# nikkolasg/playsnark

Hardware: AMD Instinct MI355X
Metric: G1 scalar-muls/s (Pippenger MSM, 2^20 pts per GPU) (higher is better)
Workload: dtype i32x14 (381-bit Fp, 28-bit unsaturated limbs, Montgomery); 1 GPU; BLS12-381 G1 MSM, 2^20 points per GPU, uniform 255-bit scalars; points_per_gpu=1048576, window_bits=20, windows=13, window_table=True, window_table_bytes=1744830464, slice=32, in_flight=4

## Files before the change

### playsnark_amd/csrc/capi.hip

```cpp
#include "../../include/playsnark_hip.h"

#include <hip/hip_runtime.h>

#include <algorithm>
#include <atomic>
#include <chrono>
#include <condition_variable>
#include <functional>
#include <mutex>
#include <cstdio>
#include <cstring>
#include <future>
#include <string>
#include <thread>
#include <vector>

#include "msm.hpp"
#include "point_pass_predict.hpp"
#include "msm_batch.hpp"
#include "msm_batch_plan.hpp"
#include "msm_batch_multi_plan.hpp"
#include "quotient.hpp"
#include "lagrange.hpp"
#include "ec_spmv.hpp"
// ... 12 lines not shown
}
#define HIP_TRY(expr)                                                                            \
    do {                                                                                         \
        hipError_t _e = (expr);                                                                  \
        if (_e != hipSuccess)                                                                    \
            return fail(PS_ERR_HIP, std::string(#expr) + ": " + hipGetErrorString(_e));          \
    } while (0)

#include "scope.hpp"

extern "C" const char* ps_last_error(void) { return g_last_error.c_str(); }
#define PS_STR_(x) #x
#define PS_STR(x) PS_STR_(x)
extern "C" const char* ps_version(void) { return "playsnark_hip 0.4 (gfx950), ABI " PS_STR(PS_ABI_VERSION); }
extern "C" int ps_abi_version(void) { return PS_ABI_VERSION; }
extern "C" int ps_device_count(void) {
    int n = 0;
    if (hipGetDeviceCount(&n) != hipSuccess) return 0;
    return n;
}

struct DevBuf {
    void* p = nullptr;
    size_t cap = 0;
    DevBuf() = default;
    DevBuf(const DevBuf&) = delete;
    DevBuf& operator=(const DevBuf&) = delete;
    ~DevBuf() { release(); }
    int ensure(size_t bytes) {
        if (bytes <= cap) return PS_OK;
        release();
        size_t want = bytes + bytes / 8 + 256;
        hipError_t e = hipMalloc(&p, want);
        if (e != hipSuccess) return fail(PS_ERR_HIP, std::string("hipMalloc workspace: ") + hipGetErrorString(e));
        cap = want;
        return PS_OK;
    }
    void release() {
        if (p) (void)hipFree(p);
        p = nullptr;
        cap = 0;
    }
};

constexpr size_t PS_PINNED_SLOT = 64 * sizeof(Xyzz<Fp2>) + 16;

struct MsmWorkspace {
    int device = 0;
    hipStream_t stream = nullptr;
    hipStream_t tail = nullptr;
    hipEvent_t ev_acc_local = nullptr, ev_tail_done = nullptr, ev_sort_local = nullptr;
    bool tail_used = false;
    DevBuf counts, offs, bsum, keys, ranks, vals, sorted, buckets, parts, segs, wins, heavy, hparts, coarse;
    DevBuf perm, border;
    DevBuf mb_fold, mb_out;
    void* h_pinned = nullptr;
    size_t h_pinned_cap = 0;
    hipEvent_t ev[PS_MSM_STAGES + 1] = {};
    bool ev_valid = false;
    ~MsmWorkspace() { destroy(); }
    bool created() const { return stream != nullptr; }
    int create(int dev) {
        const int rc = [&]() -> int {
            device = dev;
            HIP_TRY(hipSetDevice(device));
            HIP_TRY(hipStreamCreateWithFlags(&stream, hipStreamNonBlocking));
            int least = 0, greatest = 0;
            HIP_TRY(hipDeviceGetStreamPriorityRange(&least, &greatest));
            HIP_TRY(hipStreamCreateWithPriority(&tail, hipStreamNonBlocking, greatest));
            HIP_TRY(hipEventCreateWithFlags(&ev_acc_local, hipEventDisableTiming));
            HIP_TRY(hipEventCreateWithFlags(&ev_tail_done, hipEventDisableTiming));
            HIP_TRY(hipEventCreateWithFlags(&ev_sort_local, hipEventDisableTiming));
            h_pinned_cap = PS_MSM_MULTI_MAX * PS_PINNED_SLOT + 64;
            HIP_TRY(hipHostMalloc(&h_pinned, h_pinned_cap));
            for (auto& e : ev) HIP_TRY(hipEventCreate(&e));
            return PS_OK;
        }();
        if (rc) destroy();
        return rc;
    }
    int sync() {
        HIP_TRY(hipSetDevice(device));
        for (hipStream_t s : {stream, tail}) HIP_TRY(hipStreamSynchronize(s));
        return PS_OK;
    }
    void destroy() {
        for (hipStream_t s : {stream, tail}) if (s) (void)hipStreamSynchronize(s);
        for (auto& e : ev) if (e) { (void)hipEventDestroy(e); e = nullptr; }
        for (hipEvent_t* e : {&ev_acc_local, &ev_tail_done, &ev_sort_local}) if (*e) { (void)hipEventDestroy(*e); *e = nullptr; }
        if (h_pinned) (void)hipHostFree(h_pinned);
        h_pinned = nullptr;
        for (hipStream_t* s : {&tail, &stream}) if (*s) { (void)hipStreamDestroy(*s); *s = nullptr; }
    }
};

constexpr int PS_WORKERS = 6;
constexpr int PS_RING_WORKERS[4] = {2, 0, 1, 3};
constexpr int PS_LAUNCH_WORKERS[PS_WORKERS] = {0, 1, 2, 3, 4, 5};

struct ps_ctx : MsmWorkspace {
    int batch_chunk = 0;
    int batch_table = 0;
    hipEvent_t mb_ev[2] = {nullptr, nullptr};
    DevBuf pb_x, pb_y, pb_small;
    hipEvent_t pb_ev[6] = {nullptr, nullptr, nullptr, nullptr, nullptr, nullptr};
    bool pb_timed = false;
// ... 781 lines not shown
}

template <class F>
static int points_sum_t(const uint8_t* pts, size_t k, uint8_t* out, size_t wb) {
    typedef typename HostField<F>::type H;
    Xyzz<H> acc = xyzz_identity<H>();
    for (size_t i = 0; i < k; i++) {
        Affine<F> a;
        if (!read_affine(a, pts + wb * i)) return fail(PS_ERR_ENCODING, "ps_points_sum: bad point encoding");
        if (!affine_is_identity<F>(a)) { Affine<H> h = affine_to_host<F>(a); xyzz_madd<H>(acc, h.x, h.y); }
    }
    write_affine(out, acc);
    return PS_OK;
}
template <class F>
static int point_convert_t(int in_fmt, int out_fmt, const uint8_t* in, uint8_t* out, size_t wb) {
    Affine<F> a;
    bool ok = in_fmt == PS_FMT_AFFINE ? read_affine(a, in) : decompress_point(a, in);
    if (!ok) return fail(PS_ERR_ENCODING, "ps_point_convert: bad point encoding");
    if (out_fmt == PS_FMT_COMPRESSED) {
        compress_point(out, a);
        return PS_OK;
    }
    if (affine_is_identity<F>(a)) { memset(out, 0, wb); out[0] = 0x40; return PS_OK; }
    write_affine(out, xyzz_from_affine<F>(a.x, a.y));
    return PS_OK;
}
extern "C" int ps_point_convert(int group, int in_fmt, int out_fmt, const uint8_t* in, uint8_t* out) {
    if (!in || !out) return fail(PS_ERR_ARG, "ps_point_convert: NULL argument");
    if ((in_fmt != PS_FMT_AFFINE && in_fmt != PS_FMT_COMPRESSED) || (out_fmt != PS_FMT_AFFINE && out_fmt != PS_FMT_COMPRESSED))
        return fail(PS_ERR_ARG, "ps_point_convert: bad format");
    if (group == PS_G1) return point_convert_t<Fp>(in_fmt, out_fmt, in, out, 96);
    if (group == PS_G2) return point_convert_t<Fp2>(in_fmt, out_fmt, in, out, 192);
    return fail(PS_ERR_ARG, "bad group");
}
extern "C" int ps_points_sum(int group, const uint8_t* pts, size_t k, uint8_t* out) {
    if ((k && !pts) || !out) return fail(PS_ERR_ARG, "ps_points_sum: NULL argument");
    if (group == PS_G1) return points_sum_t<Fp>(pts, k, out, 96);
    if (group == PS_G2) return points_sum_t<Fp2>(pts, k, out, 192);
    return fail(PS_ERR_ARG, "bad group");
}

#define PS_STAGE_MARK(w) do { if (timed) HIP_TRY(hipEventRecord((w)->ev[evi++], st)); } while (0)
static int msm_sort(MsmWorkspace* ws, const ps_scalars* sc, const MsmPlan& pl, bool timed, hipStream_t st) {
    const size_t n = sc->n;
    const u64 total = (u64)pl.W * n;
    const u64 G = pl.G;
    const u32 scan_tiles = (u32)((G + SCAN_TILE - 1) / SCAN_TILE);
    int rc;
    if ((rc = ws->counts.ensure(4 * G))) return rc;
    if ((rc = ws->offs.ensure(4 * (G + 1)))) return rc;
    if ((rc = ws->bsum.ensure(4 * (size_t)scan_tiles + 4))) return rc;
    if ((rc = ws->keys.ensure(4 * total))) return rc;
    if ((rc = ws->ranks.ensure(4 * total))) return rc;
    if ((rc = ws->vals.ensure(4 * total))) return rc;
    if ((rc = ws->sorted.ensure(4 * total + 4))) return rc;
    if (ws->tail_used) HIP_TRY(hipStreamWaitEvent(st, ws->ev_tail_done, 0));
    if (storage_wait_ready(sc->st, st)) return fail(PS_ERR_HIP, "msm: event wait failed");
    int evi = 0;
    PS_STAGE_MARK(ws);
    DigitConst cadd{};
    for (int w = 0; w + 1 < pl.W; w++) {
        int bit = w * pl.c + pl.c - 1;
        if (bit < 256) cadd.w[bit >> 5] |= 1u << (bit & 31);
    }
    const dim3 dgrid((unsigned)((n + DIGITS_CHUNK - 1) / DIGITS_CHUNK), (unsigned)pl.W);
    const int fold_neg = sc->neg_small ? 1 : 0, single = pl.sets == 1 ? 1 : 0;
    if (G <= SORT_MAX_BUCKETS) {
        int fb = 5;
        while (((G + (1ull << fb) - 1) >> fb) > SORT_MAX_COARSE) fb++;
#if defined(PS_TAIL_TUNE)
        if (const char* e = getenv("PS_T_FB")) fb = std::max(fb, std::min(atoi(e), 10));
#endif
        const u32 ncoarse = (u32)((G + (1ull << fb) - 1) >> fb);
        if ((rc = ws->coarse.ensure(4 * (4 * (size_t)SORT_MAX_COARSE + 8)))) return rc;
        u32* coarse_cnt = (u32*)ws->coarse.p;
        u32* coarse_off = coarse_cnt + SORT_MAX_COARSE + 1;
        u32* coarse_cur = coarse_off + SORT_MAX_COARSE + 1;
        u32* tile_base = coarse_cur + SORT_MAX_COARSE + 1;
        HIP_TRY(hipMemsetAsync(coarse_cnt, 0, 4 * SORT_MAX_COARSE, st));
        const bool may_have_big_bins = total > SORT_BIG;
        if (may_have_big_bins) HIP_TRY(hipMemsetAsync(ws->counts.p, 0, 4 * G, st));
        const dim3 cgrid((unsigned)((n + (size_t)COUNT_PER_THREAD * DIGITS_THREADS - 1) / ((size_t)COUNT_PER_THREAD * DIGITS_THREADS)));
        hipLaunchKernelGGL(k_sort_count, cgrid, dim3(DIGITS_THREADS), 0, st, scalars_ptr(sc), (u32)n, pl.c, pl.W, pl.NB, cadd, fold_neg,
                           single, ncoarse, fb, (u32*)ws->ranks.p, coarse_cnt);
        PS_STAGE_MARK(ws);
        hipLaunchKernelGGL(k_sort_scan, dim3(1), dim3(SORT_MAX_COARSE), 0, st, (const u32*)coarse_cnt, ncoarse, coarse_off, coarse_cur,
                           (u32*)ws->offs.p + G, tile_base);
        hipLaunchKernelGGL(k_sort_partition, dgrid, dim3(DIGITS_THREADS), 2 * DIGITS_CHUNK * sizeof(u32), st, (const u32*)ws->ranks.p,
                           (u32)n, pl.NB, single, fb, coarse_cur, (unsigned short*)ws->keys.p, (u32*)ws->vals.p);
        PS_STAGE_MARK(ws);
        hipLaunchKernelGGL(k_sort_fine, dim3(ncoarse), dim3(SORT_FINE), 0, st, (const unsigned short*)ws->keys.p, (const u32*)ws->vals.p,
                           (const u32*)coarse_off, (u32)G, fb, (u32*)ws->offs.p, (u32*)ws->sorted.p);
        const unsigned big_grid = (unsigned)std::min<u64>(2048, total / SORT_TILE + 1);
        if (may_have_big_bins) {
        hipLaunchKernelGGL(k_sort_big_count, dim3(big_grid), dim3(SORT_FINE), 0, st, (const unsigned short*)ws->keys.p, (const u32*)coarse_off,
                           (const u32*)tile_base, ncoarse, fb, (u32*)ws->counts.p);
        hipLaunchKernelGGL(k_sort_big_scan, dim3(ncoarse), dim3(SORT_FINE), 0, st, (const u32*)coarse_off, (u32)G, fb, (u32*)ws->counts.p,
                           (u32*)ws->offs.p);
        hipLaunchKernelGGL(k_sort_big_scatter, dim3(big_grid), dim3(SORT_FINE), 0, st, (const unsigned short*)ws->keys.p,
                           (const u32*)ws->vals.p, (const u32*)coarse_off, (const u32*)tile_base, ncoarse, fb, (u32*)ws->counts.p,
                           (u32*)ws->sorted.p);
        }
    } else {
        HIP_TRY(hipMemsetAsync(ws->counts.p, 0, 4 * G, st));
        {
            int bin_shift = 4;
            while ((pl.NB >> bin_shift) > (u32)DIGITS_BINS) bin_shift++;
            hipLaunchKernelGGL(k_digits_grouped, dgrid, dim3(DIGITS_THREADS), 2 * DIGITS_CHUNK * sizeof(u32), st, scalars_ptr(sc),
                               (u32)n, pl.c, pl.W, pl.NB, cadd, bin_shift, fold_neg, single, (u32*)ws->counts.p, (u32*)ws->keys.p,
                               (u32*)ws->vals.p, (u32*)ws->ranks.p);
        }
        PS_STAGE_MARK(ws);
        hipLaunchKernelGGL(k_scan_blocks, dim3(scan_tiles), dim3(SCAN_BLOCK), 0, st, (const u32*)ws->counts.p, (u32*)ws->offs.p,
                           (u32*)ws->bsum.p, (u64)G);
        hipLaunchKernelGGL(k_scan_top, dim3(1), dim3(1024), 0, st, (u32*)ws->bsum.p, scan_tiles, (u32*)ws->offs.p + G);
        hipLaunchKernelGGL(k_scan_add, dim3(scan_tiles), dim3(SCAN_BLOCK), 0, st, (u32*)ws->offs.p, (const u32*)ws->bsum.p, (u64)G);
        PS_STAGE_MARK(ws);
        hipLaunchKernelGGL(k_scatter, dim3(nblocks(total)), dim3(256), 0, st, (const u32*)ws->keys.p, (const u32*)ws->vals.p,
                           (const u32*)ws->ranks.p, (const u32*)ws->offs.p, total, (u32*)ws->sorted.p);
    }
    if (pl.acc != ACC_SLICES) {
        if ((rc = ws->perm.ensure(4 * G))) return rc;
        if ((rc = ws->border.ensure(4 * (2 * (size_t)BO_CLASSES + 4)))) return rc;
        u32* hist = (u32*)ws->border.p;
        u32* cursors = hist + BO_CLASSES;
        u32* verdict = cursors + BO_CLASSES;
        const unsigned tiles = (unsigned)((G + BO_PLACE_TILE - 1) / BO_PLACE_TILE);
        HIP_TRY(hipMemsetAsync(hist, 0, 4 * BO_CLASSES, st));
        hipLaunchKernelGGL(k_bo_count, dim3(tiles), dim3(256), 0, st, (const u32*)ws->offs.p, (u32)G, hist);
        hipLaunchKernelGGL(k_bo_scan, dim3(1), dim3(BO_CLASSES), 0, st, (const u32*)hist, (const u32*)ws->offs.p, (u32)G, (u32)pl.acc, cursors,
                           verdict);
        hipLaunchKernelGGL(k_bo_place, dim3(tiles), dim3(256), 0, st, (const u32*)ws->offs.p, (u32)G, cursors, (u32*)ws->perm.p);
        HIP_TRY(hipMemcpyAsync((char*)ws->h_pinned + ws->h_pinned_cap - 16, verdict, 4, hipMemcpyDeviceToHost, st));
    }
    PS_STAGE_MARK(ws);
    HIP_TRY(hipGetLastError());
    if (!pl.qtail) HIP_TRY(hipMemcpyAsync((char*)ws->h_pinned + ws->h_pinned_cap - 8, (u32*)ws->offs.p + G, 4, hipMemcpyDeviceToHost, st));
    return PS_OK;
}

struct TableRef { const char* base; u64 stride; };
static bool table_ref(const ps_points* pts, size_t n, int wbits, int W, TableRef* out) {
    const Storage* st = pts->st;
    const size_t rb = table_row_bytes(pts->group);
    if (const void* t = st->table.load(std::memory_order_acquire)) {
        if (st->table_c == wbits && W <= st->table_W) {
            *out = TableRef{(const char*)t + pts->first * rb, (u64)st->table_stride};
            return true;
        }
    }
    if (const ViewTable* v = view_table_find(st, pts->first, n, wbits)) {
        const void* t = v->table.load(std::memory_order_acquire);
        if (t && W <= v->W) {
            *out = TableRef{(const char*)t, (u64)v->n};
            return true;
        }
// ... 847 lines not shown
```

### playsnark_amd/csrc/msm.hpp

```cpp
#pragma once
#include "curve.hpp"
#include "fixup_class.hpp"
#include "bucket_order.hpp"

namespace ps {

#ifndef PS_TAIL_PRIO
#define PS_TAIL_PRIO 0
#endif
#if PS_TAIL_PRIO > 0
#define PS_TAIL_PRIO_HERE __builtin_amdgcn_s_setprio(PS_TAIL_PRIO)
#else
#define PS_TAIL_PRIO_HERE do { } while (0)
#endif

struct MsmPlan {
    int c;
    int W;
    u32 NB;
    u64 G;
    int M;
    int SEG;
    int sets;
    bool table;
    bool qtail;
    bool hybrid;
    bool shortsum;
    int lpb;
    int rc_s;
    bool busy;
    int acc;
};
constexpr int ENTRY_W_SHIFT = 26;

static inline MsmPlan msm_plan(size_t n, int max_bits, int forced_c) {
    MsmPlan best{};
    double best_cost = 1e300;
    for (int c = 4; c <= 20; c++) {
        if (forced_c ? c != forced_c : c > 16) continue;
        int W = max_bits / c + 1;
        double nb = (double)(1u << (c - 1));
        double cost = (double)n * W * 10.0 + W * nb * 42.0;
        if (cost < best_cost) {
            best_cost = cost;
            best.c = c;
            best.W = W;
        }
    }
    best.NB = 1u << (best.c - 1);
    best.sets = best.W;
    best.G = (u64)best.W * best.NB;
    best.M = 32;
    const u64 total = (u64)n * best.W;
    while (best.M < 1024 && total / (2 * (u64)best.M) >= (1u << 19)) best.M *= 2;
    while (best.M < 1024 && (u64)best.M * 5 * best.G < total) best.M *= 2;
    while (best.M > 8 && total / (u64)best.M < (1u << 17) && (u64)(best.M / 2) * 5 * best.G >= total) best.M /= 2;
// ... 192 lines not shown
    u32 v[SCAN_ITEMS];
    u32 s = 0;
#pragma unroll
    for (int j = 0; j < SCAN_ITEMS; j++) {
        v[j] = (base + j < n) ? in[base + j] : 0u;
        s += v[j];
    }
    u32 total;
    u32 ex = block_excl_scan(s, &total);
#pragma unroll
    for (int j = 0; j < SCAN_ITEMS; j++) {
        if (base + j < n) out[base + j] = ex;
        ex += v[j];
    }
    if (threadIdx.x == 0) bsum[blockIdx.x] = total;
}

__global__ void __launch_bounds__(1024) k_scan_top(u32* __restrict__ bsum, u32 nb, u32* __restrict__ out_total) {
    __shared__ u32 carry_s;
    if (threadIdx.x == 0) carry_s = 0;
    __syncthreads();
    for (u32 start = 0; start < nb; start += 1024) {
        u32 idx = start + threadIdx.x;
        u32 v = idx < nb ? bsum[idx] : 0u;
        u32 total;
        u32 ex = block_excl_scan(v, &total);
        u32 carry = carry_s;
        if (idx < nb) bsum[idx] = ex + carry;
        __syncthreads();
        if (threadIdx.x == 0) carry_s = carry + total;
        __syncthreads();
    }
    if (threadIdx.x == 0) *out_total = carry_s;
}

__global__ void __launch_bounds__(SCAN_BLOCK) k_scan_add(u32* __restrict__ out, const u32* __restrict__ bsum, u64 n) {
    u64 base = (u64)blockIdx.x * SCAN_TILE + (u64)threadIdx.x * SCAN_ITEMS;
    u32 add = bsum[blockIdx.x];
#pragma unroll
    for (int j = 0; j < SCAN_ITEMS; j++)
        if (base + j < n) out[base + j] += add;
}

__global__ void __launch_bounds__(256) k_scatter(const u32* __restrict__ ent_key, const u32* __restrict__ ent_val,
                                                 const u32* __restrict__ ent_rank, const u32* __restrict__ offs, u64 total,
                                                 u32* __restrict__ sorted) {
    u64 idx = (u64)blockIdx.x * blockDim.x + threadIdx.x;
    if (idx >= total) return;
    u32 key = ent_key[idx];
    if (key == 0xffffffffu) return;
    sorted[offs[key] + ent_rank[idx]] = ent_val[idx];
}

constexpr int SORT_FINE_BITS = 10;
constexpr u32 SORT_FINE = 1u << SORT_FINE_BITS;
constexpr u32 SORT_MAX_COARSE = 1024;
constexpr u64 SORT_MAX_BUCKETS = (u64)SORT_FINE * SORT_MAX_COARSE;
static_assert(DIGITS_THREADS == (int)SORT_MAX_COARSE && SORT_FINE == SORT_MAX_COARSE, "one thread per histogram bin");

__device__ inline void scalar_plus_c(const u32* __restrict__ scalars, u32 i, const DigitConst& cadd, int fold_neg, u32 (&k)[8], u32& carry,
                                     u32& flip) {
    const uint4* sp = reinterpret_cast<const uint4*>(scalars) + 2 * (size_t)i;
    uint4 a = sp[0], b = sp[1];
    k[0] = a.x; k[1] = a.y; k[2] = a.z; k[3] = a.w; k[4] = b.x; k[5] = b.y; k[6] = b.z; k[7] = b.w;
    flip = 0;
    if (fold_neg && k[7] != 0) {
        u32 borrow = 0;
#pragma unroll
        for (int q = 0; q < 8; q++) {
            u64 t = (u64)FrParams::mod(q) - k[q] - borrow;
            k[q] = (u32)t;
            borrow = (u32)(t >> 63);
        }
        flip = 0x80000000u;
    }
    carry = 0;
#pragma unroll
    for (int q = 0; q < 8; q++) {
        u64 t = (u64)k[q] + cadd.w[q] + carry;
        k[q] = (u32)t;
        carry = (u32)(t >> 32);
    }
}
__device__ inline u32 digit_from(const u32 (&k)[8], u32 carry, int c, int W, int w, u32 NB, u32 flip) {
    const u32 mask = (1u << c) - 1u;
    const int bit = w * c, li = bit >> 5, sh = bit & 31;
    const bool top = w == W - 1;
    u64 two = (u64)limb_sel8(k, li) | ((u64)limb_sel8(k, li + 1) << 32);
    if (li == 7) two |= (u64)carry << 32;
    u32 raw = top ? (u32)(two >> sh) : ((u32)(two >> sh) & mask);
    int d = top ? (int)raw : (int)raw - (int)NB;
    if (d == 0) return 0xffffffffu;
    u32 mag = d < 0 ? (u32)(-d) : (u32)d;
    return (mag - 1u) | ((d < 0 ? 0x80000000u : 0u) ^ flip);
}
__device__ inline u32 digit_code(const u32* __restrict__ scalars, u32 i, int c, int W, int w, u32 NB, const DigitConst& cadd,
                                 int fold_neg) {
    u32 k[8], carry, flip;
    scalar_plus_c(scalars, i, cadd, fold_neg, k, carry, flip);
    return digit_from(k, carry, c, W, w, NB, flip);
}

__device__ inline void lds_count(u32* ctr, u32 bin, bool active) {
    const unsigned long long act = __ballot(active);
    if (!act) return;
    const int leader = __ffsll((long long)act) - 1;
    const u32 lb = __shfl(bin, leader, 64);
    const bool mine = active && bin == lb;
    const unsigned long long same = __ballot(mine);
    if (__popcll(same) >= 8) {
        if ((int)(threadIdx.x & 63) == leader) atomicAdd(&ctr[lb], (u32)__popcll(same));
        if (active && !mine) atomicAdd(&ctr[bin], 1u);
    } else if (active) {
        atomicAdd(&ctr[bin], 1u);
    }
}
__device__ inline u32 lds_rank(u32* ctr, u32 bin, bool active) {
    const unsigned long long act = __ballot(active);
    if (!act) return 0;
    const int lane = (int)(threadIdx.x & 63);
    const int leader = __ffsll((long long)act) - 1;
    const u32 lb = __shfl(bin, leader, 64);
    const bool mine = active && bin == lb;
    const unsigned long long same = __ballot(mine);
    u32 pos = 0;
    if (__popcll(same) >= 8) {
        u32 b0 = 0;
        if (lane == leader) b0 = atomicAdd(&ctr[lb], (u32)__popcll(same));
        b0 = __shfl(b0, leader, 64);
        if (mine) pos = b0 + (u32)__popcll(same & ((1ull << lane) - 1ull));
        else if (active) pos = atomicAdd(&ctr[bin], 1u);
    } else if (active) {
        pos = atomicAdd(&ctr[bin], 1u);
    }
    return pos;
}

constexpr int COUNT_PER_THREAD = 2;
__global__ void __launch_bounds__(DIGITS_THREADS) k_sort_count(const u32* __restrict__ scalars, u32 n, int c, int W, u32 NB,
                                                               DigitConst cadd, int fold_neg, int single_set, u32 ncoarse, int fb,
                                                               u32* __restrict__ codes, u32* __restrict__ coarse_cnt) {
    PS_TAIL_PRIO_HERE;
    __shared__ u32 hist[SORT_MAX_COARSE];
    const u32 tid = threadIdx.x;
    hist[tid] = 0;
    __syncthreads();
    for (int j = 0; j < COUNT_PER_THREAD; j++) {
        const u32 i = (blockIdx.x * COUNT_PER_THREAD + (u32)j) * DIGITS_THREADS + tid;
        const bool in = i < n;
        u32 k[8], carry = 0, flip = 0;
        if (in) scalar_plus_c(scalars, i, cadd, fold_neg, k, carry, flip);
        for (int w = 0; w < W; w++) {
            u32 code = 0xffffffffu;
            if (in) {
                code = digit_from(k, carry, c, W, w, NB, flip);
                codes[(size_t)w * n + i] = code;
            }
            const u32 key_base = single_set ? 0u : (u32)w * NB;
            lds_count(hist, (key_base + (code & 0x7fffffffu)) >> fb, code != 0xffffffffu);
        }
    }
    __syncthreads();
    if (tid < ncoarse && hist[tid]) atomicAdd(&coarse_cnt[tid], hist[tid]);
}

constexpr u32 SORT_BIG = 1u << 16;
constexpr u32 SORT_TILE = 1u << 14;

__global__ void __launch_bounds__(SORT_MAX_COARSE) k_sort_scan(const u32* __restrict__ coarse_cnt, u32 ncoarse, u32* __restrict__ coarse_off,
                                                               u32* __restrict__ coarse_cur, u32* __restrict__ offs_total,
                                                               u32* __restrict__ tile_base) {
    PS_TAIL_PRIO_HERE;
    const u32 tid = threadIdx.x;
    const u32 cnt = tid < ncoarse ? coarse_cnt[tid] : 0u;
    u32 total;
    const u32 ex = block_excl_scan(cnt, &total);
    if (tid < ncoarse) { coarse_off[tid] = ex; coarse_cur[tid] = ex; }
    if (tid == 0) { coarse_off[ncoarse] = total; *offs_total = total; }
    __syncthreads();
    const u32 tiles = cnt > SORT_BIG ? (cnt + SORT_TILE - 1) / SORT_TILE : 0u;
    u32 ttotal;
    const u32 tex = block_excl_scan(tiles, &ttotal);
    if (tid < ncoarse) tile_base[tid] = tex;
    if (tid == 0) tile_base[ncoarse] = ttotal;
}

__global__ void __launch_bounds__(DIGITS_THREADS, 8) k_sort_partition(const u32* __restrict__ codes, u32 n, u32 NB, int single_set, int fb,
                                                                   u32* __restrict__ coarse_cur, unsigned short* __restrict__ part_key,
                                                                   u32* __restrict__ part_val) {
    PS_TAIL_PRIO_HERE;
    __shared__ u32 hist[SORT_MAX_COARSE], binstart[SORT_MAX_COARSE], gbase[SORT_MAX_COARSE];
    __shared__ u32 wtot[DIGITS_THREADS / 64];
    extern __shared__ __align__(16) unsigned char dg_smem[];
    u32* lkey = reinterpret_cast<u32*>(dg_smem);
    u32* lval = lkey + DIGITS_CHUNK;
    const int w = blockIdx.y;
    const u32 chunk_base = blockIdx.x * DIGITS_CHUNK;
    const u32 tid = threadIdx.x;
    hist[tid] = 0;
    __syncthreads();
    const u32 key_base = single_set ? 0u : (u32)w * NB;
    const u32 wtag = single_set ? (u32)w << ENTRY_W_SHIFT : 0u;
    u32 dig[DIGITS_PER_THREAD];
#pragma unroll
    for (int j = 0; j < DIGITS_PER_THREAD; j++) {
        const u32 i = chunk_base + j * DIGITS_THREADS + tid;
        const u32 code = i < n ? codes[(size_t)w * n + i] : 0xffffffffu;
        dig[j] = code;
        lds_count(hist, (key_base + (code & 0x7fffffffu)) >> fb, code != 0xffffffffu);
    }
    __syncthreads();
    const u32 cnt = hist[tid];
    const u32 inc = wave_incl_scan(cnt);
    if ((tid & 63) == 63) wtot[tid >> 6] = inc;
    __syncthreads();
    u32 before = 0, total = 0;
    for (int q = 0; q < DIGITS_THREADS / 64; q++) {
        const u32 t = wtot[q];
        if (q < (int)(tid >> 6)) before += t;
        total += t;
    }
    const u32 ex = before + inc - cnt;
    __syncthreads();
    binstart[tid] = ex;
    hist[tid] = ex;
    gbase[tid] = cnt ? atomicAdd(&coarse_cur[tid], cnt) : 0u;
    __syncthreads();
#pragma unroll
    for (int j = 0; j < DIGITS_PER_THREAD; j++) {
        const u32 code = dig[j];
        const bool act = code != 0xffffffffu;
        const u32 key = key_base + (code & 0x7fffffffu);
        const u32 pos = lds_rank(hist, key >> fb, act);
        if (act) {
            lkey[pos] = key;
            lval[pos] = (chunk_base + j * DIGITS_THREADS + tid) | (code & 0x80000000u) | wtag;
        }
    }
    __syncthreads();
    for (u32 p = tid; p < total; p += DIGITS_THREADS) {
        const u32 key = lkey[p], b = key >> fb;
        const u32 dst = gbase[b] + (p - binstart[b]);
        part_key[dst] = (unsigned short)(key & ((1u << fb) - 1u));
        part_val[dst] = lval[p];
    }
}

__global__ void __launch_bounds__(SORT_FINE) k_sort_fine(const unsigned short* __restrict__ part_key, const u32* __restrict__ part_val,
                                                         const u32* __restrict__ coarse_off, u32 G, int fb, u32* __restrict__ offs,
                                                         u32* __restrict__ sorted) {
    PS_TAIL_PRIO_HERE;
    __shared__ u32 hist[SORT_FINE];
    __shared__ u32 wtot[SORT_FINE / 64];
    const u32 p = blockIdx.x, tid = threadIdx.x;
    const u32 lo = coarse_off[p], hi = coarse_off[p + 1];
    if (hi - lo > SORT_BIG) return;
    hist[tid] = 0;
    __syncthreads();
    constexpr u32 UNR = 4;
    for (u32 i0 = lo; i0 < hi; i0 += UNR * SORT_FINE) {
        u32 k[UNR];
        bool act[UNR];
#pragma unroll
        for (u32 u = 0; u < UNR; u++) {
            const u32 i = i0 + u * SORT_FINE + tid;
            act[u] = i < hi;
            k[u] = act[u] ? (u32)part_key[i] : 0u;
        }
#pragma unroll
        for (u32 u = 0; u < UNR; u++) lds_count(hist, k[u], act[u]);
    }
    __syncthreads();
    const u32 cnt = hist[tid];
    const u32 inc = wave_incl_scan(cnt);
    if ((tid & 63) == 63) wtot[tid >> 6] = inc;
    __syncthreads();
    u32 before = 0;
    for (int q = 0; q < (int)(tid >> 6); q++) before += wtot[q];
    const u32 start = lo + before + inc - cnt;
    const u32 g = (p << fb) + tid;
    if (tid < (1u << fb) && g < G) offs[g] = start;
    __syncthreads();
    hist[tid] = start;
    __syncthreads();
    for (u32 i0 = lo; i0 < hi; i0 += UNR * SORT_FINE) {
        u32 k[UNR], v[UNR];
        bool act[UNR];
#pragma unroll
        for (u32 u = 0; u < UNR; u++) {
            const u32 i = i0 + u * SORT_FINE + tid;
            act[u] = i < hi;
            k[u] = act[u] ? (u32)part_key[i] : 0u;
            v[u] = act[u] ? part_val[i] : 0u;
        }
#pragma unroll
        for (u32 u = 0; u < UNR; u++) {
            const u32 pos = lds_rank(hist, k[u], act[u]);
            if (act[u]) sorted[pos] = v[u];
        }
    }
}

__device__ inline bool sort_big_tile(u32 t, const u32* __restrict__ tile_base, const u32* __restrict__ coarse_off, u32 ncoarse,
                                     u32* p_out, u32* lo_out, u32* hi_out) {
    if (t >= tile_base[ncoarse]) return false;
    u32 lo = 0, hi = ncoarse;
    while (hi - lo > 1) {
        const u32 mid = (lo + hi) >> 1;
        if (tile_base[mid] <= t) lo = mid; else hi = mid;
    }
    while (tile_base[lo + 1] <= t) lo++;
    const u32 first = coarse_off[lo] + (t - tile_base[lo]) * SORT_TILE, end = coarse_off[lo + 1];
    *p_out = lo;
    *lo_out = first;
    *hi_out = end - first > SORT_TILE ? first + SORT_TILE : end;
    return true;
}
constexpr u32 SORT_TILE_PER_THREAD = SORT_TILE / SORT_FINE;

__global__ void __launch_bounds__(SORT_FINE) k_sort_big_count(const unsigned short* __restrict__ part_key, const u32* __restrict__ coarse_off,
                                                              const u32* __restrict__ tile_base, u32 ncoarse, int fb,
                                                              u32* __restrict__ gcnt) {
    PS_TAIL_PRIO_HERE;
    __shared__ u32 hist[SORT_FINE];
    const u32 tid = threadIdx.x;
    for (u32 t = blockIdx.x;; t += gridDim.x) {
        u32 p, lo, hi;
        if (!sort_big_tile(t, tile_base, coarse_off, ncoarse, &p, &lo, &hi)) return;
        hist[tid] = 0;
        __syncthreads();
#pragma unroll 4
        for (u32 j = 0; j < SORT_TILE_PER_THREAD; j++) {
            const u32 i = lo + j * SORT_FINE + tid;
            const bool act = i < hi;
            lds_count(hist, act ? (u32)part_key[i] : 0u, act);
        }
        __syncthreads();
        if (tid < (1u << fb) && hist[tid]) atomicAdd(&gcnt[((size_t)p << fb) + tid], hist[tid]);
        __syncthreads();
    }
}
__global__ void __launch_bounds__(SORT_FINE) k_sort_big_scan(const u32* __restrict__ coarse_off, u32 G, int fb, u32* __restrict__ gcnt,
                                                             u32* __restrict__ offs) {
    PS_TAIL_PRIO_HERE;
    __shared__ u32 wtot[SORT_FINE / 64];
    const u32 p = blockIdx.x, tid = threadIdx.x;
    const u32 lo = coarse_off[p], hi = coarse_off[p + 1];
    if (hi - lo <= SORT_BIG) return;
    const u32 g = (p << fb) + tid;
    const bool own = tid < (1u << fb) && g < G;
    const u32 cnt = own ? gcnt[g] : 0u;
    const u32 inc = wave_incl_scan(cnt);
    if ((tid & 63) == 63) wtot[tid >> 6] = inc;
    __syncthreads();
    u32 before = 0;
    for (int q = 0; q < (int)(tid >> 6); q++) before += wtot[q];
    const u32 start = lo + before + inc - cnt;
    if (own) { offs[g] = start; gcnt[g] = start; }
}
__global__ void __launch_bounds__(SORT_FINE) k_sort_big_scatter(const unsigned short* __restrict__ part_key, const u32* __restrict__ part_val,
                                                                const u32* __restrict__ coarse_off, const u32* __restrict__ tile_base,
                                                                u32 ncoarse, int fb, u32* __restrict__ gcur, u32* __restrict__ sorted) {
    PS_TAIL_PRIO_HERE;
    __shared__ u32 hist[SORT_FINE];
    const u32 tid = threadIdx.x;
    for (u32 t = blockIdx.x;; t += gridDim.x) {
        u32 p, lo, hi;
        if (!sort_big_tile(t, tile_base, coarse_off, ncoarse, &p, &lo, &hi)) return;
        hist[tid] = 0;
        __syncthreads();
        u32 k[SORT_TILE_PER_THREAD];
#pragma unroll
        for (u32 j = 0; j < SORT_TILE_PER_THREAD; j++) {
            const u32 i = lo + j * SORT_FINE + tid;
            const bool act = i < hi;
            k[j] = act ? (u32)part_key[i] : 0xffffffffu;
            lds_count(hist, act ? k[j] : 0u, act);
        }
        __syncthreads();
        const u32 cnt = hist[tid];
        __syncthreads();
        hist[tid] = (tid < (1u << fb) && cnt) ? atomicAdd(&gcur[((size_t)p << fb) + tid], cnt) : 0u;
        __syncthreads();
#pragma unroll
        for (u32 j = 0; j < SORT_TILE_PER_THREAD; j++) {
            const bool act = k[j] != 0xffffffffu;
            const u32 pos = lds_rank(hist, act ? k[j] : 0u, act);
            if (act) sorted[pos] = part_val[lo + j * SORT_FINE + tid];
        }
        __syncthreads();
    }
}

template <class KF> struct FieldTraits { typedef KF Store; static constexpr int LANES = 1; };
template <> struct FieldTraits<Fp2s> { typedef Fp2 Store; static constexpr int LANES = 2; };
template <class S> struct KernelField { typedef S type; };
template <> struct KernelField<Fp2> { typedef Fp2s type; };

__device__ inline Fp ld_f(const Fp* p, const Fp*) { return *p; }
__device__ inline void st_f(Fp* p, const Fp& v) { *p = v; }
__device__ inline Fp2s ld_f(const Fp2* p, const Fp2s*) { return Fp2s{pair_lane() ? p->c1 : p->c0}; }
__device__ inline void st_f(Fp2* p, const Fp2s& v) { if (pair_lane()) p->c1 = v.v; else p->c0 = v.v; }

template <class KF>
__device__ inline Affine<KF> ld_affine(const Affine<typename FieldTraits<KF>::Store>* p) {
    Affine<KF> r;
    r.x = ld_f(&p->x, (const KF*)0);
    r.y = ld_f(&p->y, (const KF*)0);
    return r;
}
template <class KF>
__device__ inline Xyzz<KF> ld_xyzz(const Xyzz<typename FieldTraits<KF>::Store>* p) {
    Xyzz<KF> r;
    r.x = ld_f(&p->x, (const KF*)0);
    r.y = ld_f(&p->y, (const KF*)0);
    r.zz = ld_f(&p->zz, (const KF*)0);
    r.zzz = ld_f(&p->zzz, (const KF*)0);
    return r;
}
template <class KF>
__device__ inline void st_xyzz(Xyzz<typename FieldTraits<KF>::Store>* p, const Xyzz<KF>& v) {
    st_f(&p->x, v.x);
    st_f(&p->y, v.y);
    st_f(&p->zz, v.zz);
    st_f(&p->zzz, v.zzz);
}
template <class KF> __device__ inline u32 logical_tid() { return (blockIdx.x * blockDim.x + threadIdx.x) / FieldTraits<KF>::LANES; }
template <class KF> __device__ inline u32 logical_local() { return threadIdx.x / FieldTraits<KF>::LANES; }
template <class KF> __device__ inline u32 logical_block() { return blockDim.x / FieldTraits<KF>::LANES; }
template <class KF> __device__ inline bool pair_leader() { return FieldTraits<KF>::LANES == 1 || pair_lane() == 0; }

template <class KF>
__device__ inline void block_tree_sum(Xyzz<typename FieldTraits<KF>::Store>* sm, const Xyzz<KF>& mine) {
    const u32 lt = logical_local<KF>();
    st_xyzz<KF>(&sm[lt], mine);
    __syncthreads();
    for (u32 stride = logical_block<KF>() >> 1; stride > 0; stride >>= 1) {
        if (lt < stride) {
            Xyzz<KF> a = ld_xyzz<KF>(&sm[lt]), b = ld_xyzz<KF>(&sm[lt + stride]);
            xyzz_add_inl<KF>(a, b);
            st_xyzz<KF>(&sm[lt], a);
// ... 843 lines not shown
```

Measured before the change: 470.8 million G1 scalar-muls/s.

## Recompute scalar digits in partition with per-tile histograms instead of staging codes

The coarse sort no longer writes W*n digit codes to global memory in the count pass and rereads them in partition. Both passes now work on scalar tiles, recompute digits from the scalars, and record a per-tile coarse histogram. A new tile-scan kernel turns those histograms into deterministic per-tile offsets, which replaces the global atomic cursor. This saves memory traffic and atomics but adds a second digit extraction and a tiles×ncoarse histogram buffer that must be written, scanned and reread.

```diff
diff --git a/playsnark_amd/csrc/capi.hip b/playsnark_amd/csrc/capi.hip
--- a/playsnark_amd/csrc/capi.hip
+++ b/playsnark_amd/csrc/capi.hip
@@ -88,6 +88,7 @@
     hipEvent_t ev_acc_local = nullptr, ev_tail_done = nullptr, ev_sort_local = nullptr;
     bool tail_used = false;
     DevBuf counts, offs, bsum, keys, ranks, vals, sorted, buckets, parts, segs, wins, heavy, hparts, coarse;
+    DevBuf tile_hist, tile_off;
     DevBuf perm, border;
     DevBuf mb_fold, mb_out;
     void* h_pinned = nullptr;
@@ -975,7 +976,6 @@
     if ((rc = ws->offs.ensure(4 * (G + 1)))) return rc;
     if ((rc = ws->bsum.ensure(4 * (size_t)scan_tiles + 4))) return rc;
     if ((rc = ws->keys.ensure(4 * total))) return rc;
-    if ((rc = ws->ranks.ensure(4 * total))) return rc;
     if ((rc = ws->vals.ensure(4 * total))) return rc;
     if ((rc = ws->sorted.ensure(4 * total + 4))) return rc;
     if (ws->tail_used) HIP_TRY(hipStreamWaitEvent(st, ws->ev_tail_done, 0));
@@ -990,28 +990,30 @@
     const dim3 dgrid((unsigned)((n + DIGITS_CHUNK - 1) / DIGITS_CHUNK), (unsigned)pl.W);
     const int fold_neg = sc->neg_small ? 1 : 0, single = pl.sets == 1 ? 1 : 0;
     if (G <= SORT_MAX_BUCKETS) {
-        int fb = 5;
-        while (((G + (1ull << fb) - 1) >> fb) > SORT_MAX_COARSE) fb++;
+        int fb = sort_fine_bits(G);
 #if defined(PS_TAIL_TUNE)
         if (const char* e = getenv("PS_T_FB")) fb = std::max(fb, std::min(atoi(e), 10));
 #endif
-        const u32 ncoarse = (u32)((G + (1ull << fb) - 1) >> fb);
+        const u32 ncoarse = sort_ncoarse(G, fb);
+        const u32 T = sort_tile_scalars(pl.W), tiles = sort_tile_count(n, T);
+        if ((rc = ws->tile_hist.ensure(4 * sort_tile_words(tiles, ncoarse)))) return rc;
+        if ((rc = ws->tile_off.ensure(4 * sort_tile_words(tiles, ncoarse)))) return rc;
         if ((rc = ws->coarse.ensure(4 * (4 * (size_t)SORT_MAX_COARSE + 8)))) return rc;
         u32* coarse_cnt = (u32*)ws->coarse.p;
         u32* coarse_off = coarse_cnt + SORT_MAX_COARSE + 1;
-        u32* coarse_cur = coarse_off + SORT_MAX_COARSE + 1;
-        u32* tile_base = coarse_cur + SORT_MAX_COARSE + 1;
-        HIP_TRY(hipMemsetAsync(coarse_cnt, 0, 4 * SORT_MAX_COARSE, st));
+        u32* tile_base = coarse_off + SORT_MAX_COARSE + 1;
         const bool may_have_big_bins = total > SORT_BIG;
         if (may_have_big_bins) HIP_TRY(hipMemsetAsync(ws->counts.p, 0, 4 * G, st));
-        const dim3 cgrid((unsigned)((n + (size_t)COUNT_PER_THREAD * DIGITS_THREADS - 1) / ((size_t)COUNT_PER_THREAD * DIGITS_THREADS)));
-        hipLaunchKernelGGL(k_sort_count, cgrid, dim3(DIGITS_THREADS), 0, st, scalars_ptr(sc), (u32)n, pl.c, pl.W, pl.NB, cadd, fold_neg,
-                           single, ncoarse, fb, (u32*)ws->ranks.p, coarse_cnt);
+        hipLaunchKernelGGL(k_sort_count, dim3(tiles), dim3(DIGITS_THREADS), 0, st, scalars_ptr(sc), (u32)n, pl.c, pl.W, pl.NB, cadd, fold_neg,
+                           single, ncoarse, fb, T, (u32*)ws->tile_hist.p);
         PS_STAGE_MARK(ws);
-        hipLaunchKernelGGL(k_sort_scan, dim3(1), dim3(SORT_MAX_COARSE), 0, st, (const u32*)coarse_cnt, ncoarse, coarse_off, coarse_cur,
+        hipLaunchKernelGGL(k_sort_tile_scan, dim3(sort_tscan_grid(ncoarse)), dim3(SORT_TSCAN_BINS * SORT_TSCAN_SEGS), 0, st,
+                           (const u32*)ws->tile_hist.p, tiles, ncoarse, (u32*)ws->tile_off.p, coarse_cnt);
+        hipLaunchKernelGGL(k_sort_scan, dim3(1), dim3(SORT_MAX_COARSE), 0, st, (const u32*)coarse_cnt, ncoarse, coarse_off, (u32*)nullptr,
                            (u32*)ws->offs.p + G, tile_base);
-        hipLaunchKernelGGL(k_sort_partition, dgrid, dim3(DIGITS_THREADS), 2 * DIGITS_CHUNK * sizeof(u32), st, (const u32*)ws->ranks.p,
-                           (u32)n, pl.NB, single, fb, coarse_cur, (unsigned short*)ws->keys.p, (u32*)ws->vals.p);
+        hipLaunchKernelGGL(k_sort_partition, dim3(tiles), dim3(DIGITS_THREADS), SORT_TILE_LDS, st, scalars_ptr(sc), (u32)n, pl.c, pl.W, pl.NB,
+                           cadd, fold_neg, single, ncoarse, fb, T, (const u32*)ws->tile_hist.p, (const u32*)ws->tile_off.p,
+                           (const u32*)coarse_off, (unsigned short*)ws->keys.p, (u32*)ws->vals.p);
         PS_STAGE_MARK(ws);
         hipLaunchKernelGGL(k_sort_fine, dim3(ncoarse), dim3(SORT_FINE), 0, st, (const unsigned short*)ws->keys.p, (const u32*)ws->vals.p,
                            (const u32*)coarse_off, (u32)G, fb, (u32*)ws->offs.p, (u32*)ws->sorted.p);
@@ -1026,6 +1028,7 @@
                            (u32*)ws->sorted.p);
         }
     } else {
+        if ((rc = ws->ranks.ensure(4 * total))) return rc;
         HIP_TRY(hipMemsetAsync(ws->counts.p, 0, 4 * G, st));
         {
             int bin_shift = 4;
diff --git a/playsnark_amd/csrc/msm.hpp b/playsnark_amd/csrc/msm.hpp
--- a/playsnark_amd/csrc/msm.hpp
+++ b/playsnark_amd/csrc/msm.hpp
@@ -2,6 +2,7 @@
 #include "curve.hpp"
 #include "fixup_class.hpp"
 #include "bucket_order.hpp"
+#include "sort_tiles.hpp"
 
 namespace ps {
 
@@ -300,11 +301,8 @@
     sorted[offs[key] + ent_rank[idx]] = ent_val[idx];
 }
 
-constexpr int SORT_FINE_BITS = 10;
-constexpr u32 SORT_FINE = 1u << SORT_FINE_BITS;
-constexpr u32 SORT_MAX_COARSE = 1024;
-constexpr u64 SORT_MAX_BUCKETS = (u64)SORT_FINE * SORT_MAX_COARSE;
 static_assert(DIGITS_THREADS == (int)SORT_MAX_COARSE && SORT_FINE == SORT_MAX_COARSE, "one thread per histogram bin");
+static_assert(SORT_PARTITION_STATIC_LDS == 2 * 4 * SORT_MAX_COARSE + 4 * (DIGITS_THREADS / 64), "k_sort_partition's static LDS");
 
 __device__ inline void scalar_plus_c(const u32* __restrict__ scalars, u32 i, const DigitConst& cadd, int fold_neg, u32 (&k)[8], u32& carry,
                                      u32& flip) {
@@ -387,29 +385,61 @@
 constexpr int COUNT_PER_THREAD = 2;
 __global__ void __launch_bounds__(DIGITS_THREADS) k_sort_count(const u32* __restrict__ scalars, u32 n, int c, int W, u32 NB,
                                                                DigitConst cadd, int fold_neg, int single_set, u32 ncoarse, int fb,
-                                                               u32* __restrict__ codes, u32* __restrict__ coarse_cnt) {
+                                                               u32 T, u32* __restrict__ tile_hist) {
     PS_TAIL_PRIO_HERE;
     __shared__ u32 hist[SORT_MAX_COARSE];
     const u32 tid = threadIdx.x;
     hist[tid] = 0;
     __syncthreads();
-    for (int j = 0; j < COUNT_PER_THREAD; j++) {
-        const u32 i = (blockIdx.x * COUNT_PER_THREAD + (u32)j) * DIGITS_THREADS + tid;
-        const bool in = i < n;
+    const u64 first = sort_tile_first(blockIdx.x, T);
+    for (u32 s0 = 0; s0 < T; s0 += DIGITS_THREADS) {
+        const u32 s_wave = s0 + (tid & ~63u);
+        if (s_wave >= T || first + s_wave >= n) continue;
+        const u64 i64 = first + s0 + tid;
+        const bool in = s0 + tid < T && i64 < n;
+        const u32 i = (u32)i64;
         u32 k[8], carry = 0, flip = 0;
         if (in) scalar_plus_c(scalars, i, cadd, fold_neg, k, carry, flip);
         for (int w = 0; w < W; w++) {
-            u32 code = 0xffffffffu;
-            if (in) {
-                code = digit_from(k, carry, c, W, w, NB, flip);
-                codes[(size_t)w * n + i] = code;
-            }
+            const u32 code = in ? digit_from(k, carry, c, W, w, NB, flip) : 0xffffffffu;
             const u32 key_base = single_set ? 0u : (u32)w * NB;
             lds_count(hist, (key_base + (code & 0x7fffffffu)) >> fb, code != 0xffffffffu);
         }
     }
     __syncthreads();
-    if (tid < ncoarse && hist[tid]) atomicAdd(&coarse_cnt[tid], hist[tid]);
+    if (tid < ncoarse) tile_hist[(size_t)blockIdx.x * ncoarse + tid] = hist[tid];
+}
+
+__global__ void __launch_bounds__(SORT_TSCAN_BINS * SORT_TSCAN_SEGS) k_sort_tile_scan(const u32* __restrict__ tile_hist, u32 tiles,
+                                                                                      u32 ncoarse, u32* __restrict__ tile_off,
+                                                                                      u32* __restrict__ coarse_cnt) {
+    PS_TAIL_PRIO_HERE;
+    __shared__ u32 segsum[SORT_TSCAN_SEGS][SORT_TSCAN_BINS];
+    const u32 b = threadIdx.x % SORT_TSCAN_BINS, seg = threadIdx.x / SORT_TSCAN_BINS;
+    const u32 bin = blockIdx.x * SORT_TSCAN_BINS + b;
+    const bool ok = bin < ncoarse;
+    const u32 t0 = sort_tscan_first(seg, tiles), t1 = sort_tscan_end(seg, tiles);
+    u32 sum = 0;
+    if (ok) {
+#pragma unroll 8
+        for (u32 t = t0; t < t1; t++) sum += tile_hist[(size_t)t * ncoarse + bin];
+    }
+    segsum[seg][b] = sum;
+    __syncthreads();
+    u32 run = 0, total = 0;
+    for (u32 q = 0; q < SORT_TSCAN_SEGS; q++) {
+        const u32 v = segsum[q][b];
+        if (q < seg) run += v;
+        total += v;
+    }
+    if (!ok) return;
+    if (seg == 0) coarse_cnt[bin] = total;
+#pragma unroll 8
+    for (u32 t = t0; t < t1; t++) {
+        const size_t at = (size_t)t * ncoarse + bin;
+        tile_off[at] = run;
+        run += tile_hist[at];
+    }
 }
 
 constexpr u32 SORT_BIG = 1u << 16;
@@ -423,7 +453,10 @@
     const u32 cnt = tid < ncoarse ? coarse_cnt[tid] : 0u;
     u32 total;
     const u32 ex = block_excl_scan(cnt, &total);
-    if (tid < ncoarse) { coarse_off[tid] = ex; coarse_cur[tid] = ex; }
+    if (tid < ncoarse) {
+        coarse_off[tid] = ex;
+        if (coarse_cur) coarse_cur[tid] = ex;
+    }
     if (tid == 0) { coarse_off[ncoarse] = total; *offs_total = total; }
     __syncthreads();
     const u32 tiles = cnt > SORT_BIG ? (cnt + SORT_TILE - 1) / SORT_TILE : 0u;
@@ -433,32 +466,20 @@
     if (tid == 0) tile_base[ncoarse] = ttotal;
 }
 
-__global__ void __launch_bounds__(DIGITS_THREADS, 8) k_sort_partition(const u32* __restrict__ codes, u32 n, u32 NB, int single_set, int fb,
-                                                                   u32* __restrict__ coarse_cur, unsigned short* __restrict__ part_key,
-                                                                   u32* __restrict__ part_val) {
+__global__ void __launch_bounds__(DIGITS_THREADS, 8) k_sort_partition(const u32* __restrict__ scalars, u32 n, int c, int W, u32 NB,
+                                                                   DigitConst cadd, int fold_neg, int single_set, u32 ncoarse, int fb,
+                                                                   u32 T, const u32* __restrict__ tile_hist,
+                                                                   const u32* __restrict__ tile_off, const u32* __restrict__ coarse_off,
+                                                                   unsigned short* __restrict__ part_key, u32* __restrict__ part_val) {
     PS_TAIL_PRIO_HERE;
-    __shared__ u32 hist[SORT_MAX_COARSE], binstart[SORT_MAX_COARSE], gbase[SORT_MAX_COARSE];
+    __shared__ u32 hist[SORT_MAX_COARSE], gdelta[SORT_MAX_COARSE];
     __shared__ u32 wtot[DIGITS_THREADS / 64];
     extern __shared__ __align__(16) unsigned char dg_smem[];
     u32* lkey = reinterpret_cast<u32*>(dg_smem);
-    u32* lval = lkey + DIGITS_CHUNK;
-    const int w = blockIdx.y;
-    const u32 chunk_base = blockIdx.x * DIGITS_CHUNK;
+    u32* lval = lkey + SORT_TILE_ENTRIES;
     const u32 tid = threadIdx.x;
-    hist[tid] = 0;
-    __syncthreads();
-    const u32 key_base = single_set ? 0u : (u32)w * NB;
-    const u32 wtag = single_set ? (u32)w << ENTRY_W_SHIFT : 0u;
-    u32 dig[DIGITS_PER_THREAD];
-#pragma unroll
-    for (int j = 0; j < DIGITS_PER_THREAD; j++) {
-        const u32 i = chunk_base + j * DIGITS_THREADS + tid;
-        const u32 code = i < n ? codes[(size_t)w * n + i] : 0xffffffffu;
-        dig[j] = code;
-        lds_count(hist, (key_base + (code & 0x7fffffffu)) >> fb, code != 0xffffffffu);
-    }
-    __syncthreads();
-    const u32 cnt = hist[tid];
+    const size_t row = (size_t)blockIdx.x * ncoarse;
+    const u32 cnt = tid < ncoarse ? tile_hist[row + tid] : 0u;
     const u32 inc = wave_incl_scan(cnt);
     if ((tid & 63) == 63) wtot[tid >> 6] = inc;
     __syncthreads();
@@ -469,26 +490,33 @@
         total += t;
     }
     const u32 ex = before + inc - cnt;
-    __syncthreads();
-    binstart[tid] = ex;
     hist[tid] = ex;
-    gbase[tid] = cnt ? atomicAdd(&coarse_cur[tid], cnt) : 0u;
-    __syncthreads();
-#pragma unroll
-    for (int j = 0; j < DIGITS_PER_THREAD; j++) {
-        const u32 code = dig[j];
-        const bool act = code != 0xffffffffu;
-        const u32 key = key_base + (code & 0x7fffffffu);
-        const u32 pos = lds_rank(hist, key >> fb, act);
-        if (act) {
-            lkey[pos] = key;
-            lval[pos] = (chunk_base + j * DIGITS_THREADS + tid) | (code & 0x80000000u) | wtag;
+    gdelta[tid] = cnt ? coarse_off[tid] + tile_off[row + tid] - ex : 0u;
+    __syncthreads();
+    const u64 first = sort_tile_first(blockIdx.x, T);
+    for (u32 s0 = 0; s0 < T; s0 += DIGITS_THREADS) {
+        const u32 s_wave = s0 + (tid & ~63u);
+        if (s_wave >= T || first + s_wave >= n) continue;
+        const u64 i64 = first + s0 + tid;
+        const bool in = s0 + tid < T && i64 < n;
+        const u32 i = (u32)i64;
+        u32 k[8], carry = 0, flip = 0;
+        if (in) scalar_plus_c(scalars, i, cadd, fold_neg, k, carry, flip);
+        for (int w = 0; w < W; w++) {
+            const u32 code = in ? digit_from(k, carry, c, W, w, NB, flip) : 0xffffffffu;
+            const bool act = code != 0xffffffffu;
+            const u32 key = (single_set ? 0u : (u32)w * NB) + (code & 0x7fffffffu);
+            const u32 pos = lds_rank(hist, key >> fb, act);
+            if (act) {
+                lkey[pos] = key;
+                lval[pos] = i | (code & 0x80000000u) | (single_set ? (u32)w << ENTRY_W_SHIFT : 0u);
+            }
         }
     }
     __syncthreads();
     for (u32 p = tid; p < total; p += DIGITS_THREADS) {
         const u32 key = lkey[p], b = key >> fb;
-        const u32 dst = gbase[b] + (p - binstart[b]);
+        const u32 dst = gdelta[b] + p;
         part_key[dst] = (unsigned short)(key & ((1u << fb) - 1u));
         part_val[dst] = lval[p];
     }
diff --git a/playsnark_amd/csrc/sort_tiles.hpp b/playsnark_amd/csrc/sort_tiles.hpp
--- /dev/null
+++ b/playsnark_amd/csrc/sort_tiles.hpp
@@ -0,0 +1,58 @@
+#pragma once
+#include <cstddef>
+
+#include "field.hpp"
+
+namespace ps {
+
+constexpr int SORT_FINE_BITS = 10;
+constexpr u32 SORT_FINE = 1u << SORT_FINE_BITS;
+constexpr u32 SORT_MAX_COARSE = 1024;
+constexpr u64 SORT_MAX_BUCKETS = (u64)SORT_FINE * SORT_MAX_COARSE;
+
+PS_HD inline int sort_fine_bits(u64 G) {
+    int fb = 5;
+    while (fb < SORT_FINE_BITS && ((G + (1ull << fb) - 1) >> fb) > SORT_MAX_COARSE) fb++;
+    return fb;
+}
+PS_HD inline u32 sort_ncoarse(u64 G, int fb) { return (u32)((G + (1ull << fb) - 1) >> fb); }
+
+#ifndef PS_SORT_TILE_LDS
+#define PS_SORT_TILE_LDS 72704
+#endif
+constexpr u32 SORT_TILE_LDS = PS_SORT_TILE_LDS;
+constexpr u32 SORT_PARTITION_STATIC_LDS = 2 * 4 * SORT_MAX_COARSE + 64;
+constexpr u32 SORT_CU_LDS = 160 * 1024;
+static_assert(SORT_TILE_LDS % 8 == 0 && SORT_TILE_LDS + SORT_PARTITION_STATIC_LDS <= SORT_CU_LDS, "the staging area fits a CU");
+constexpr u32 SORT_ENTRY_LDS = 2 * sizeof(u32);
+constexpr u32 SORT_TILE_ENTRIES = SORT_TILE_LDS / SORT_ENTRY_LDS;
+constexpr int SORT_MAX_WINDOWS = 64;
+static_assert(SORT_TILE_ENTRIES >= (u32)SORT_MAX_WINDOWS, "a tile holds at least one scalar's digits");
+
+PS_HD inline u32 sort_tile_scalars(int W) {
+    const u32 w = W < 1 ? 1u : (u32)W;
+    const u32 t = SORT_TILE_ENTRIES / w;
+    return t ? t : 1u;
+}
+PS_HD inline u32 sort_tile_count(u64 n, u32 T) { return (u32)((n + T - 1) / T); }
+PS_HD inline u64 sort_tile_first(u32 t, u32 T) { return (u64)t * T; }
+PS_HD inline u64 sort_tile_end(u32 t, u32 T, u64 n) {
+    const u64 e = (u64)(t + 1) * T;
+    return e < n ? e : n;
+}
+PS_HD inline size_t sort_tile_words(u32 tiles, u32 ncoarse) { return (size_t)tiles * ncoarse; }
+
+constexpr u32 SORT_TSCAN_BINS = 4;
+constexpr u32 SORT_TSCAN_SEGS = 64;
+PS_HD inline u32 sort_tscan_grid(u32 ncoarse) { return (ncoarse + SORT_TSCAN_BINS - 1) / SORT_TSCAN_BINS; }
+PS_HD inline u32 sort_tscan_per(u32 tiles) { return (tiles + SORT_TSCAN_SEGS - 1) / SORT_TSCAN_SEGS; }
+PS_HD inline u32 sort_tscan_first(u32 seg, u32 tiles) {
+    const u64 f = (u64)seg * sort_tscan_per(tiles);
+    return f < tiles ? (u32)f : tiles;
+}
+PS_HD inline u32 sort_tscan_end(u32 seg, u32 tiles) {
+    const u64 e = (u64)sort_tscan_first(seg, tiles) + sort_tscan_per(tiles);
+    return e < tiles ? (u32)e : tiles;
+}
+
+}
```

Result: slower. 463.6 million G1 scalar-muls/s (-1.5%).

## Record per-element ranks during counting pass to skip second LDS rank pass in sorts

Applied to the files above, without the earlier changes.

In the partition, fine and big-scatter sort kernels, the counting pass now computes each element's rank within its bin with lds_rank and keeps it in registers (packed beside the key or two per register). The scatter pass then places each element at the bin start plus the stored rank, so the second round of LDS atomics is no longer needed. k_sort_fine gets a register-resident single-walk path for bins of up to SORT_FINE_KEEP*SORT_FINE elements and now declares a minimum occupancy of 8 in its launch bounds. The cost is extra register pressure, mainly the 32-entry kr array. Placement also stays stable only if lds_rank hands out ranks in the same order as before.

```diff
diff --git a/playsnark_amd/csrc/msm.hpp b/playsnark_amd/csrc/msm.hpp
--- a/playsnark_amd/csrc/msm.hpp
+++ b/playsnark_amd/csrc/msm.hpp
@@ -414,6 +414,8 @@
 
 constexpr u32 SORT_BIG = 1u << 16;
 constexpr u32 SORT_TILE = 1u << 14;
+constexpr u32 SORT_FINE_KEEP = 32;
+static_assert(SORT_FINE_KEEP * SORT_FINE <= (1u << (32 - SORT_FINE_BITS)) && SORT_FINE_KEEP * SORT_FINE <= SORT_BIG, "rank beside the key");
 
 __global__ void __launch_bounds__(SORT_MAX_COARSE) k_sort_scan(const u32* __restrict__ coarse_cnt, u32 ncoarse, u32* __restrict__ coarse_off,
                                                                u32* __restrict__ coarse_cur, u32* __restrict__ offs_total,
@@ -449,13 +451,16 @@
     __syncthreads();
     const u32 key_base = single_set ? 0u : (u32)w * NB;
     const u32 wtag = single_set ? (u32)w << ENTRY_W_SHIFT : 0u;
+    static_assert(DIGITS_CHUNK <= (1 << 16) && DIGITS_PER_THREAD % 2 == 0, "two ranks per register");
     u32 dig[DIGITS_PER_THREAD];
+    u32 rk[DIGITS_PER_THREAD / 2];
 #pragma unroll
     for (int j = 0; j < DIGITS_PER_THREAD; j++) {
         const u32 i = chunk_base + j * DIGITS_THREADS + tid;
         const u32 code = i < n ? codes[(size_t)w * n + i] : 0xffffffffu;
         dig[j] = code;
-        lds_count(hist, (key_base + (code & 0x7fffffffu)) >> fb, code != 0xffffffffu);
+        const u32 r = lds_rank(hist, (key_base + (code & 0x7fffffffu)) >> fb, code != 0xffffffffu);
+        if (j & 1) rk[j >> 1] |= r << 16; else rk[j >> 1] = r;
     }
     __syncthreads();
     const u32 cnt = hist[tid];
@@ -469,9 +474,7 @@
         total += t;
     }
     const u32 ex = before + inc - cnt;
-    __syncthreads();
     binstart[tid] = ex;
-    hist[tid] = ex;
     gbase[tid] = cnt ? atomicAdd(&coarse_cur[tid], cnt) : 0u;
     __syncthreads();
 #pragma unroll
@@ -479,8 +482,8 @@
         const u32 code = dig[j];
         const bool act = code != 0xffffffffu;
         const u32 key = key_base + (code & 0x7fffffffu);
-        const u32 pos = lds_rank(hist, key >> fb, act);
         if (act) {
+            const u32 pos = binstart[key >> fb] + ((rk[j >> 1] >> (16 * (j & 1))) & 0xffffu);
             lkey[pos] = key;
             lval[pos] = (chunk_base + j * DIGITS_THREADS + tid) | (code & 0x80000000u) | wtag;
         }
@@ -494,7 +497,7 @@
     }
 }
 
-__global__ void __launch_bounds__(SORT_FINE) k_sort_fine(const unsigned short* __restrict__ part_key, const u32* __restrict__ part_val,
+__global__ void __launch_bounds__(SORT_FINE, 8) k_sort_fine(const unsigned short* __restrict__ part_key, const u32* __restrict__ part_val,
                                                          const u32* __restrict__ coarse_off, u32 G, int fb, u32* __restrict__ offs,
                                                          u32* __restrict__ sorted) {
     PS_TAIL_PRIO_HERE;
@@ -506,17 +509,36 @@
     hist[tid] = 0;
     __syncthreads();
     constexpr u32 UNR = 4;
-    for (u32 i0 = lo; i0 < hi; i0 += UNR * SORT_FINE) {
-        u32 k[UNR];
-        bool act[UNR];
-#pragma unroll
-        for (u32 u = 0; u < UNR; u++) {
-            const u32 i = i0 + u * SORT_FINE + tid;
-            act[u] = i < hi;
-            k[u] = act[u] ? (u32)part_key[i] : 0u;
-        }
-#pragma unroll
-        for (u32 u = 0; u < UNR; u++) lds_count(hist, k[u], act[u]);
+    const bool one_walk = hi - lo <= SORT_FINE_KEEP * SORT_FINE;
+    u32 kr[SORT_FINE_KEEP];
+    if (one_walk) {
+#pragma unroll
+        for (u32 t = 0; t < SORT_FINE_KEEP; t += UNR) {
+            if (lo + t * SORT_FINE >= hi) continue;
+            u32 k[UNR];
+            bool act[UNR];
+#pragma unroll
+            for (u32 u = 0; u < UNR; u++) {
+                const u32 i = lo + (t + u) * SORT_FINE + tid;
+                act[u] = i < hi;
+                k[u] = act[u] ? (u32)part_key[i] : 0u;
+            }
+#pragma unroll
+            for (u32 u = 0; u < UNR; u++) kr[t + u] = k[u] | lds_rank(hist, k[u], act[u]) << SORT_FINE_BITS;
+        }
+    } else {
+        for (u32 i0 = lo; i0 < hi; i0 += UNR * SORT_FINE) {
+            u32 k[UNR];
+            bool act[UNR];
+#pragma unroll
+            for (u32 u = 0; u < UNR; u++) {
+                const u32 i = i0 + u * SORT_FINE + tid;
+                act[u] = i < hi;
+                k[u] = act[u] ? (u32)part_key[i] : 0u;
+            }
+#pragma unroll
+            for (u32 u = 0; u < UNR; u++) lds_count(hist, k[u], act[u]);
+        }
     }
     __syncthreads();
     const u32 cnt = hist[tid];
@@ -531,6 +553,24 @@
     __syncthreads();
     hist[tid] = start;
     __syncthreads();
+    if (one_walk) {
+#pragma unroll
+        for (u32 t = 0; t < SORT_FINE_KEEP; t += UNR) {
+            if (lo + t * SORT_FINE >= hi) continue;
+            u32 v[UNR];
+            bool act[UNR];
+#pragma unroll
+            for (u32 u = 0; u < UNR; u++) {
+                const u32 i = lo + (t + u) * SORT_FINE + tid;
+                act[u] = i < hi;
+                v[u] = act[u] ? part_val[i] : 0u;
+            }
+#pragma unroll
+            for (u32 u = 0; u < UNR; u++)
+                if (act[u]) sorted[hist[kr[t + u] & (SORT_FINE - 1u)] + (kr[t + u] >> SORT_FINE_BITS)] = v[u];
+        }
+        return;
+    }
     for (u32 i0 = lo; i0 < hi; i0 += UNR * SORT_FINE) {
         u32 k[UNR], v[UNR];
         bool act[UNR];
@@ -622,8 +662,9 @@
         for (u32 j = 0; j < SORT_TILE_PER_THREAD; j++) {
             const u32 i = lo + j * SORT_FINE + tid;
             const bool act = i < hi;
-            k[j] = act ? (u32)part_key[i] : 0xffffffffu;
-            lds_count(hist, act ? k[j] : 0u, act);
+            const u32 key = act ? (u32)part_key[i] : 0u;
+            const u32 r = lds_rank(hist, key, act);
+            k[j] = act ? key | r << SORT_FINE_BITS : 0xffffffffu;
         }
         __syncthreads();
         const u32 cnt = hist[tid];
@@ -632,9 +673,7 @@
         __syncthreads();
 #pragma unroll
         for (u32 j = 0; j < SORT_TILE_PER_THREAD; j++) {
-            const bool act = k[j] != 0xffffffffu;
-            const u32 pos = lds_rank(hist, act ? k[j] : 0u, act);
-            if (act) sorted[pos] = part_val[lo + j * SORT_FINE + tid];
+            if (k[j] != 0xffffffffu) sorted[hist[k[j] & (SORT_FINE - 1u)] + (k[j] >> SORT_FINE_BITS)] = part_val[lo + j * SORT_FINE + tid];
         }
         __syncthreads();
     }
```

Measured after the change: 459.0 million G1 scalar-muls/s before, 458.5 million G1 scalar-muls/s after, median of 3. Within noise of the previous version (-0.1%).
